# denix56/SI-Mamba

Measured on AMD Instinct MI355X. Metric: point-clouds/sec (fwd+bwd), higher is better.
Workload: dtype f32; 1 GPU; PointMamba classifier train step (FPS+kNN grouping, encoder, spectral SAST ordering, 12 Mamba blocks d=384 at L=1024, head, AdamW), 1024 pts -> 128 patches; global_batch=64, per_gpu_batch=64, npoints=1024, patches=128, mamba_seq_len=1024, parallelism=dp1, communicator_ranks=1, library_gemm=tuned solution table (si_mamba_amd/tuned/gemm_gfx950.csv)

## Files before the change

### include/simamba.h

```cpp
#ifndef SIMAMBA_H_
#define SIMAMBA_H_

#include <stddef.h>

#ifdef __cplusplus
extern "C" {
#endif

#define SIMAMBA_ABI_VERSION 9

#define SIMAMBA_F32  0
#define SIMAMBA_BF16 1

#define SIMAMBA_OK            0
#define SIMAMBA_E_NULLPTR    -1
#define SIMAMBA_E_SHAPE      -2
#define SIMAMBA_E_DTYPE      -3
#define SIMAMBA_E_DSTATE     -4
#define SIMAMBA_E_WIDTH      -5
#define SIMAMBA_E_WORKSPACE  -6
#define SIMAMBA_E_GROUPS     -7
#define SIMAMBA_E_ALIGN      -8
#define SIMAMBA_E_VARIANT    -9

#define SIMAMBA_SCAN_CHUNK 128

#define SIMAMBA_SCAN_CKPT_ROW 128
#define SIMAMBA_SCAN_CKPT_SEQ 16

int         simamba_abi_version(void);
const char* simamba_strerror(int rc);
int         simamba_scan_num_chunks(int seqlen);
int         simamba_scan_fwd_auto_variant(int batch, int dim);
int         simamba_scan_ckpt_step(int batch, int dim, int seqlen, int dstate, int io_dtype);
long long   simamba_scan_ckpt_floats(int batch, int dim, int seqlen, int dstate, int ckpt_step);

#define SIMAMBA_SCAN_AUTO    0
#define SIMAMBA_SCAN_ROWSCAN 1
#define SIMAMBA_SCAN_LPC2    2
#define SIMAMBA_SCAN_LPC4    4
#define SIMAMBA_SCAN_MIX     6
int simamba_selective_scan_fwd(const void* u, const void* delta, const float* A,
                               const void* B, const void* C, const float* D, const void* z,
                               const float* delta_bias, void* out, float* x_ckpt,
                               float* last_state, int batch, int dim, int seqlen, int dstate,
                               int io_dtype, int delta_softplus, long long z_bstride,
                               long long bc_bstride, long long bc_nstride, long long bc_tstride,
                               int ckpt_step, int variant, void* stream);

int simamba_selective_scan_bwd(const void* u, const void* delta, const float* A,
                               const void* B, const void* C, const float* D, const void* z,
                               const float* delta_bias, const void* dout, const float* x_ckpt,
                               void* du, void* ddelta, float* dA, float* dB, float* dC,
                               float* dD, void* dz, float* ddelta_bias,
                               int batch, int dim, int seqlen, int dstate,
                               int io_dtype, int delta_softplus, long long z_bstride,
                               long long dz_bstride, long long bc_bstride, long long bc_nstride,
                               long long bc_tstride, int ckpt_step, void* stream);

int simamba_selective_scan_dt_fwd(const void* u, const void* xdbl, const void* wdt, const float* A, const float* D,
                                  const void* z, const float* delta_bias, void* out, float* x_ckpt, float* last_state,
                                  int batch, int dim, int seqlen, int dstate, int dt_rank, int io_dtype,
                                  long long z_bstride, long long xdbl_bstride, long long xdbl_tstride, int ckpt_step,
                                  int variant, void* stream);
int simamba_selective_scan_dt_bwd(const void* u, const void* xdbl, const void* wdt, const float* A, const float* D,
                                  const void* z, const float* delta_bias, const void* dout, const float* x_ckpt,
                                  void* du, void* ddelta, float* dA, float* dB, float* dC, float* dD, void* dz,
                                  float* ddelta_bias, int batch, int dim, int seqlen, int dstate, int dt_rank,
                                  int io_dtype, long long z_bstride, long long dz_bstride, long long xdbl_bstride,
                                  long long xdbl_tstride, void* stream);

int simamba_xdt_proj_fwd(const void* x, const void* wx, const void* wdt, void* xdbl, void* delta,
                         int batch, int D, int seqlen, int S, int R, int io_dtype, long long x_bstride,
                         void* stream);
int simamba_conv_xdt_proj_fwd(const void* x, const float* cw, const float* cb, const void* wx, const void* wdt,
                              void* xconv, void* xdbl, void* delta, int batch, int D, int seqlen, int S, int R,
                              int io_dtype, long long x_bstride, void* stream);

int simamba_seq_gather_fwd(const void* in, const int* idx, void* out, int batch, int channels, int G, int L,
                           long long out_bstride, int io_dtype, void* stream);
int simamba_seq_gather_bwd(const void* dout, const int* inv, void* din, int batch, int channels, int G, int L,
                           int R, long long dout_bstride, int io_dtype, void* stream);

int simamba_causal_conv1d_fwd(const void* x, const float* w, const float* bias, void* out,
                              int batch, int dim, int seqlen, int width, int silu,
                              int io_dtype, long long x_bstride, void* stream);
int simamba_causal_conv1d_bwd(const void* x, const float* w, const float* bias,
                              const void* dout, void* dx, float* dw, float* dbias,
                              int batch, int dim, int seqlen, int width, int silu,
                              int io_dtype, long long x_bstride, long long dx_bstride, void* stream);

int simamba_add_layer_norm_grid(int batch, int rows_per_batch);
int simamba_add_layer_norm_fwd(const void* hidden, const float* residual, const float* rowscale,
                               const float* weight, const float* bias, float* residual_out,
                               void* normed, float* mean, float* rstd, int batch, int rows_per_batch,
                               int dim, float eps, int hidden_dtype, int out_dtype, void* stream);
int simamba_add_layer_norm_bwd(const void* dnormed, const float* dresidual_out,
                               const float* residual_out, const float* mean, const float* rstd,
                               const float* weight, const float* rowscale, float* dresidual,
                               void* dhidden, float* dwb_partial, int batch, int rows_per_batch,
                               int dim, int hidden_dtype, int out_dtype, void* stream);

int simamba_out_proj_add_ln_fwd(const void* y, const void* w, const float* residual, const float* rowscale,
                                const float* gamma, const float* beta, float* residual_out, void* normed, float* mean,
                                float* rstd, int batch, int K, int L, int C, float eps, int out_dtype, void* stream);

int simamba_in_proj_fwd(const void* x, const void* w, void* xz, int batch, int L, int C, int M, int io_dtype,
                        void* stream);

int simamba_bn_relu_grid(long long rows);
int simamba_bn_relu_fwd(const void* x, const float* gterm, int group, const float* weight, const float* bias,
                        float* running_mean, float* running_var, float momentum, float eps, int training,
                        void* y, float* mean, float* invstd, float* partial, long long rows, int C,
                        long long ld, int io_dtype, void* stream);
int simamba_bn_relu_bwd(const void* dy, const void* x, const float* gterm, int group, const float* weight,
                        const float* bias, const float* mean, const float* invstd, void* dx, float* dgterm,
                        int dgroup, float* dweight, float* dbias, float* partial, long long rows, int C,
                        long long ld, int io_dtype, int training, void* stream);
int simamba_group_max_fwd(const void* x, void* out, unsigned char* idx, long long groups, int n, int C,
                          int io_dtype, void* stream);
int simamba_group_max_bwd(const void* dout, const unsigned char* idx, void* dx, long long groups, int n, int C,
                          int io_dtype, void* stream);

int simamba_three_nn(const float* xyz1, const float* xyz2, int* idx, float* weight, int batch, int N, int S,
                     void* stream);
int simamba_three_interpolate_fwd(const void* feats, const int* idx, const float* weight, void* out, int batch,
                                  int N, int S, int C, int io_dtype, void* stream);
int simamba_three_interpolate_bwd(const void* dout, const int* idx, const float* weight, float* dfeats, int batch,
                                  int N, int S, int C, int io_dtype, void* stream);

int simamba_chamfer_fwd(const float* pred, const float* gt, float* dist, unsigned char* idx1, unsigned char* idx2,
                        long long pairs, int n, int m, void* stream);
int simamba_chamfer_bwd(const float* pred, const float* gt, const float* ddist, const unsigned char* idx1,
                        const unsigned char* idx2, float* dpred, long long pairs, int n, int m, void* stream);

int simamba_knn_group(const float* points, const float* centers, long long* idx, int batch, int N, int G, int K,
                      void* stream);

#define SIMAMBA_SPEC_SYMMETRIC   0x01u
#define SIMAMBA_SPEC_SELF_LOOP   0x02u
#define SIMAMBA_SPEC_BINARY      0x04u
#define SIMAMBA_SPEC_MATRIX_SYM  0x08u
#define SIMAMBA_SPEC_SMALLEST    0x10u
#define SIMAMBA_SPEC_SIGMA_MEAN  0x20u

int simamba_knn_graph(const float* points, float* adj, void* workspace, size_t ws_bytes,
                      int B, int G, int F, int knn, float alpha, unsigned flags, void* stream);

int simamba_laplacian_topk(const float* adj, float* evals, float* evecs, long long* order,
                           float* all_evals, float* all_evecs, int B, int G, int k,
                           unsigned flags, void* stream);

size_t simamba_spectral_workspace_bytes(int B, int G);

int simamba_spectral_topk(const float* centers, float* evals, float* evecs, long long* order,
                          void* workspace, size_t ws_bytes, int B, int G, int knn, float alpha,
                          int k, unsigned flags, void* stream);

int simamba_farthest_point_sample(const float* points, long long* idx, float* centers, int B, int N,
                                  int K, void* stream);

int simamba_argsort_rows(const float* vals, long long* idx, int rows, int n, void* stream);

#ifdef __cplusplus
}
#endif
#endif
```

### si_mamba_amd/_lib.py

```python
from __future__ import annotations

import ctypes
import os
from ctypes import c_char_p, c_float, c_int, c_longlong, c_size_t, c_uint, c_void_p

_HERE = os.path.dirname(os.path.abspath(__file__))
LIB_PATH = os.path.join(_HERE, "libsimamba_hip.so")

F32, BF16 = 0, 1

SPEC_SYMMETRIC = 0x01
SPEC_SELF_LOOP = 0x02
SPEC_BINARY = 0x04
SPEC_MATRIX_SYM = 0x08
SPEC_SMALLEST = 0x10
SPEC_SIGMA_MEAN = 0x20

SCAN_AUTO, SCAN_ROWSCAN, SCAN_LPC2, SCAN_LPC4, SCAN_MIX = 0, 1, 2, 4, 6
CKPT_ROW, CKPT_SEQ = 128, 16

_P = c_void_p
_LL = c_longlong
ABI_VERSION = 9
SIGNATURES = {
    "simamba_abi_version": (c_int, []),
    "simamba_strerror": (c_char_p, [c_int]),
    "simamba_scan_num_chunks": (c_int, [c_int]),
    "simamba_scan_fwd_auto_variant": (c_int, [c_int, c_int]),
    "simamba_scan_ckpt_step": (c_int, [c_int, c_int, c_int, c_int, c_int]),
    "simamba_scan_ckpt_floats": (_LL, [c_int, c_int, c_int, c_int, c_int]),
    "simamba_selective_scan_fwd": (c_int, [_P, _P, _P, _P, _P, _P, _P, _P, _P, _P, _P,
                                           c_int, c_int, c_int, c_int, c_int, c_int,
                                           _LL, _LL, _LL, _LL, c_int, c_int, _P]),
    "simamba_selective_scan_bwd": (c_int, [_P, _P, _P, _P, _P, _P, _P, _P, _P, _P,
                                           _P, _P, _P, _P, _P, _P, _P, _P,
                                           c_int, c_int, c_int, c_int, c_int, c_int,
                                           _LL, _LL, _LL, _LL, _LL, c_int, _P]),
    "simamba_selective_scan_dt_fwd": (c_int, [_P, _P, _P, _P, _P, _P, _P, _P, _P, _P,
                                              c_int, c_int, c_int, c_int, c_int, c_int,
                                              _LL, _LL, _LL, c_int, c_int, _P]),
    "simamba_selective_scan_dt_bwd": (c_int, [_P, _P, _P, _P, _P, _P, _P, _P, _P,
                                              _P, _P, _P, _P, _P, _P, _P, _P,
                                              c_int, c_int, c_int, c_int, c_int, c_int,
                                              _LL, _LL, _LL, _LL, _P]),
    "simamba_xdt_proj_fwd": (c_int, [_P, _P, _P, _P, _P, c_int, c_int, c_int, c_int, c_int, c_int, _LL, _P]),
    "simamba_conv_xdt_proj_fwd": (c_int, [_P, _P, _P, _P, _P, _P, _P, _P, c_int, c_int, c_int, c_int, c_int, c_int, _LL,
                                          _P]),
    "simamba_seq_gather_fwd": (c_int, [_P, _P, _P, c_int, c_int, c_int, c_int, _LL, c_int, _P]),
    "simamba_seq_gather_bwd": (c_int, [_P, _P, _P, c_int, c_int, c_int, c_int, c_int, _LL, c_int, _P]),
    "simamba_causal_conv1d_fwd": (c_int, [_P, _P, _P, _P, c_int, c_int, c_int, c_int, c_int, c_int, _LL, _P]),
    "simamba_causal_conv1d_bwd": (c_int, [_P, _P, _P, _P, _P, _P, _P,
                                          c_int, c_int, c_int, c_int, c_int, c_int, _LL, _LL, _P]),
    "simamba_add_layer_norm_grid": (c_int, [c_int, c_int]),
    "simamba_add_layer_norm_fwd": (c_int, [_P, _P, _P, _P, _P, _P, _P, _P, _P, c_int, c_int, c_int, c_float,
                                           c_int, c_int, _P]),
    "simamba_add_layer_norm_bwd": (c_int, [_P, _P, _P, _P, _P, _P, _P, _P, _P, _P, c_int, c_int, c_int,
                                           c_int, c_int, _P]),
    "simamba_out_proj_add_ln_fwd": (c_int, [_P, _P, _P, _P, _P, _P, _P, _P, _P, _P, c_int, c_int, c_int, c_int, c_float,
                                            c_int, _P]),
    "simamba_in_proj_fwd": (c_int, [_P, _P, _P, c_int, c_int, c_int, c_int, c_int, _P]),
    "simamba_bn_relu_grid": (c_int, [_LL]),
    "simamba_bn_relu_fwd": (c_int, [_P, _P, c_int, _P, _P, _P, _P, c_float, c_float, c_int, _P, _P, _P, _P, _LL, c_int,
                                    _LL, c_int, _P]),
    "simamba_bn_relu_bwd": (c_int, [_P, _P, _P, c_int, _P, _P, _P, _P, _P, _P, c_int, _P, _P, _P, _LL, c_int, _LL,
                                    c_int, c_int, _P]),
    "simamba_group_max_fwd": (c_int, [_P, _P, _P, _LL, c_int, c_int, c_int, _P]),
    "simamba_group_max_bwd": (c_int, [_P, _P, _P, _LL, c_int, c_int, c_int, _P]),
    "simamba_three_nn": (c_int, [_P, _P, _P, _P, c_int, c_int, c_int, _P]),
    "simamba_three_interpolate_fwd": (c_int, [_P, _P, _P, _P, c_int, c_int, c_int, c_int, c_int, _P]),
    "simamba_three_interpolate_bwd": (c_int, [_P, _P, _P, _P, c_int, c_int, c_int, c_int, c_int, _P]),
    "simamba_chamfer_fwd": (c_int, [_P, _P, _P, _P, _P, _LL, c_int, c_int, _P]),
    "simamba_chamfer_bwd": (c_int, [_P, _P, _P, _P, _P, _P, _LL, c_int, c_int, _P]),
    "simamba_knn_group": (c_int, [_P, _P, _P, c_int, c_int, c_int, c_int, _P]),
    "simamba_knn_graph": (c_int, [_P, _P, _P, c_size_t, c_int, c_int, c_int, c_int, c_float, c_uint, _P]),
    "simamba_laplacian_topk": (c_int, [_P, _P, _P, _P, _P, _P, c_int, c_int, c_int, c_uint, _P]),
    "simamba_spectral_workspace_bytes": (c_size_t, [c_int, c_int]),
    "simamba_spectral_topk": (c_int, [_P, _P, _P, _P, _P, c_size_t, c_int, c_int, c_int, c_float,
                                      c_int, c_uint, _P]),
    "simamba_argsort_rows": (c_int, [_P, _P, c_int, c_int, _P]),
    "simamba_farthest_point_sample": (c_int, [_P, _P, _P, c_int, c_int, c_int, _P]),
}

_lib = None


def load():
    global _lib
    if _lib is not None:
        return _lib
    if not os.path.exists(LIB_PATH):
        raise RuntimeError(
            f"{LIB_PATH} not found: build it with `python -c 'import __graft_entry__ as g; g.build()'` "
            "or `make -C si_mamba_amd/csrc`.  si_mamba_amd has no CPU / eager fallback.")
    lib = ctypes.CDLL(LIB_PATH)
    for name, (res, args) in SIGNATURES.items():
        fn = getattr(lib, name)
        fn.restype = res
        fn.argtypes = args
    got = lib.simamba_abi_version()
    if got != ABI_VERSION:
        raise RuntimeError(f"libsimamba_hip.so ABI version {got}, binding expects {ABI_VERSION}")
    _lib = lib
    return lib


def check(rc: int, what: str):
    if rc != 0:
        msg = load().simamba_strerror(rc).decode()
        raise RuntimeError(f"{what} failed (rc={rc}): {msg}")


def ptr(t):
    return None if t is None else t.data_ptr()


def dtype_code(dtype):
    import torch
    if dtype == torch.float32:
        return F32
    if dtype == torch.bfloat16:
        return BF16
    raise TypeError(f"si_mamba_amd kernels take float32 or bfloat16 activations, got {dtype}")


def stream_ptr(device):
    import torch
    return torch.cuda.current_stream(device).cuda_stream


def require_gpu(t, what):
    if not t.is_cuda:
        raise RuntimeError(
            f"{what}: tensor is on {t.device}; si_mamba_amd runs on a ROCm device only "
            "(no CPU fallback -- the CPU restatement lives in oracle/ and is test-only)")


_timing = {"on": False, "events": {}, "only": None}


def enable_kernel_timing(on=True, only=None):
    _timing["on"] = bool(on)
    _timing["events"] = {}
    _timing["only"] = None if only is None else frozenset(only)


class timed:
    __slots__ = ("name", "dev", "ev")

    def __init__(self, name, device):
        self.name, self.dev, self.ev = name, device, None

    def __enter__(self):
        if _timing["on"] and (_timing["only"] is None or self.name in _timing["only"]):
            import torch
            a, b = torch.cuda.Event(enable_timing=True), torch.cuda.Event(enable_timing=True)
            a.record(torch.cuda.current_stream(self.dev))
            self.ev = (a, b)
        return self

    def __exit__(self, *exc):
        if self.ev is not None:
            import torch
            self.ev[1].record(torch.cuda.current_stream(self.dev))
            _timing["events"].setdefault(self.name, []).append(self.ev)
        return False


def kernel_times():
    out = {}
    for name, evs in _timing["events"].items():
        ms = [a.elapsed_time(b) for a, b in evs]
        out[name] = (len(ms), sum(ms) / max(len(ms), 1))
    return out


_scan_variant = [SCAN_AUTO]


class scan_variant:

    def __init__(self, variant):
        self.v, self.prev = int(variant), None

    def __enter__(self):
        self.prev, _scan_variant[0] = _scan_variant[0], self.v
        return self

    def __exit__(self, *exc):
        _scan_variant[0] = self.prev
        return False


def current_scan_variant():
    return _scan_variant[0]


_scan_ckpt = [0]


class scan_ckpt:

    def __init__(self, step):
        self.v, self.prev = int(step), None

    def __enter__(self):
        self.prev, _scan_ckpt[0] = _scan_ckpt[0], self.v
        return self

    def __exit__(self, *exc):
        _scan_ckpt[0] = self.prev
        return False


_fuse_dt = [None]
counters = {}


def count(name):
    counters[name] = counters.get(name, 0) + 1



class scan_fuse_dt:

    def __init__(self, on):
        self.v, self.prev = (None if on is None else bool(on)), None

    def __enter__(self):
        self.prev, _fuse_dt[0] = _fuse_dt[0], self.v
        return self

    def __exit__(self, *exc):
        _fuse_dt[0] = self.prev
        return False


def fuse_dt_enabled(dtype):
    import torch
    return (dtype == torch.bfloat16) if _fuse_dt[0] is None else _fuse_dt[0]


_fuse_out_norm = [True]
_hand_in_proj = [None]


class fuse_out_norm:

    def __init__(self, on):
        self.v, self.prev = bool(on), None

    def __enter__(self):
        self.prev, _fuse_out_norm[0] = _fuse_out_norm[0], self.v
        return self

    def __exit__(self, *exc):
        _fuse_out_norm[0] = self.prev
        return False


def fuse_out_norm_enabled():
    return _fuse_out_norm[0]


class hand_in_proj:

    def __init__(self, on):
        self.v, self.prev = (None if on is None else bool(on)), None

    def __enter__(self):
        self.prev, _hand_in_proj[0] = _hand_in_proj[0], self.v
        return self

    def __exit__(self, *exc):
        _hand_in_proj[0] = self.prev
        return False


def in_proj_hand_enabled(workgroups, dtype=None):
    import torch
    if _hand_in_proj[0] is not None:
        return _hand_in_proj[0]
    return dtype != torch.float32 and workgroups >= IN_PROJ_MIN_WORKGROUPS


IN_PROJ_MIN_WORKGROUPS = 192


def scan_plan(batch, dim, seqlen, dstate, dtype, aligned, device, need_grad):
    import torch
    lib = load()
    code = dtype_code(dtype)
    step = _scan_ckpt[0] or lib.simamba_scan_ckpt_step(batch, dim, seqlen, dstate, code)
    if step == CKPT_SEQ and not (aligned and dstate == 16 and dim % 64 == 0 and
                                 seqlen % (4 if code == F32 else 8) == 0):
        step = CKPT_ROW
    if _scan_variant[0] == SCAN_ROWSCAN:
        step = CKPT_ROW
    if not need_grad:
        return step, None
    n = lib.simamba_scan_ckpt_floats(batch, dim, seqlen, dstate, step)
    return step, (torch.empty(n, device=device, dtype=torch.float32) if n else None)


def scan_bwd_accumulators(batch, dim, seqlen, dstate, has_D, has_bias, device):
    import torch
    sizes = [dim * dstate, batch * dstate * seqlen, batch * dstate * seqlen, dim if has_D else 0,
             dim if has_bias else 0]
    flat = torch.empty(sum(sizes), device=device, dtype=torch.float32)
    parts, o = [], 0
    for n in sizes:
        parts.append(flat[o:o + n])
        o += n
    dA = parts[0].view(dim, dstate)
    dB = parts[1].view(batch, dstate, seqlen)
    dC = parts[2].view(batch, dstate, seqlen)
    return dA, dB, dC, (parts[3] if has_D else None), (parts[4] if has_bias else None)
```

### si_mamba_amd/mamba_inner.py

```python
from __future__ import annotations

import torch

from . import _lib


def _w(t, dtype):
    return t if t.dtype == dtype else t.to(dtype)


def _wx(W, X):
    return torch.bmm(W.unsqueeze(0).expand(X.shape[0], -1, -1), X)


def _xw(X, W):
    return torch.bmm(X, W.unsqueeze(0).expand(X.shape[0], -1, -1))


def _sum_bmm(X, Y):
    return torch.bmm(X, Y).sum(0, dtype=torch.float32)


class InProjFn(torch.autograd.Function):

    @staticmethod
    def forward(ctx, hidden, weight, bias):
        io = hidden.dtype
        if torch.is_autocast_enabled("cuda"):
            io = torch.get_autocast_dtype("cuda")
            hidden = hidden.to(io)
        wc = _w(weight, io)
        xz = tokens_times_weight(hidden, wc) if bias is None else _wx(wc, hidden.transpose(1, 2))
        if bias is not None:
            xz = xz + _w(bias, io)[None, :, None]
        ctx.save_for_backward(hidden, weight)
        ctx.wc = wc
        ctx.has_bias = bias is not None
        return xz

    @staticmethod
    def backward(ctx, dxz):
        hidden, weight = ctx.saved_tensors
        io = hidden.dtype
        dxz = dxz.to(io)
        dh = _xw(dxz.transpose(1, 2), ctx.wc) if ctx.needs_input_grad[0] else None
        dw = _sum_bmm(dxz, hidden).to(weight.dtype) if ctx.needs_input_grad[1] else None
        db = dxz.sum((0, 2)).to(weight.dtype) if ctx.has_bias else None
        return dh, dw, db


def tokens_times_weight(x, w):
    if (x.dtype in (torch.bfloat16, torch.float32) and w.dtype == x.dtype and x.is_cuda and x.dim() == 3
            and x.is_contiguous() and in_proj_hand_ok(x, w)):
        lib = _lib.load()
        Bsz, L, C = x.shape
        wcc = w.contiguous()
        out = torch.empty(Bsz, w.shape[0], L, device=x.device, dtype=x.dtype)
        with torch.cuda.device(x.device), _lib.timed("in_proj_fwd", x.device):
            rc = lib.simamba_in_proj_fwd(x.data_ptr(), wcc.data_ptr(), out.data_ptr(), Bsz, L, C, w.shape[0],
                                         _lib.dtype_code(x.dtype), _lib.stream_ptr(x.device))
        _lib.check(rc, "simamba_in_proj_fwd")
        _lib.count("in_proj_hand")
        return out
    return _wx(w, x.transpose(1, 2))


def in_proj_hand_ok(hidden, wc):
    Bsz, L, C = hidden.shape
    tile = 128 if hidden.dtype == torch.float32 else 256
    return (C % 64 == 0 and C <= 384 and wc.shape[0] % 32 == 0 and L % 8 == 0 and hidden.data_ptr() % 16 == 0
            and _lib.in_proj_hand_enabled(Bsz * ((L + tile - 1) // tile), hidden.dtype))


def in_proj_fn(hidden, weight, bias=None):
    return InProjFn.apply(hidden, weight, bias)


def xdt_proj_fused_ok(x, wx, wdt, conv=False):
    S, D = wx.shape
    R = wdt.shape[1]
    pack = 4 if x.dtype == torch.float32 else 8
    return (x.is_cuda and x.dtype in (torch.float32, torch.bfloat16) and wx.dtype == x.dtype and wdt.dtype == x.dtype
            and x.dim() == 3 and x.stride(2) == 1 and x.stride(1) == x.shape[2] and x.stride(0) % pack == 0
            and x.shape[1] == D and D % 64 == 0 and x.shape[2] % pack == 0 and S % 4 == 0 and S <= 64
            and D * x.shape[2] * 4 < 2 ** 32 - 65536 and (not conv or D <= 1024)
            and R % 4 == 0 and 4 <= R <= 24 and S >= R and wdt.shape[0] == D and x.data_ptr() % 16 == 0)


def xdt_proj_fwd(x, wx, wdt, conv=None, want_delta=True):
    lib = _lib.load()
    Bsz, D, L = x.shape
    S, R = wx.shape[0], wdt.shape[1]
    wxc, wdc = wx.contiguous(), wdt.contiguous()
    x_dbl = torch.empty(Bsz, L, S, device=x.device, dtype=x.dtype)
    delta = torch.empty(Bsz, D, L, device=x.device, dtype=x.dtype) if want_delta else None
    with torch.cuda.device(x.device), _lib.timed("xdt_proj_fwd", x.device):
        if conv is None:
            rc = lib.simamba_xdt_proj_fwd(x.data_ptr(), wxc.data_ptr(), wdc.data_ptr(), x_dbl.data_ptr(),
                                          _lib.ptr(delta), Bsz, D, L, S, R, _lib.dtype_code(x.dtype), x.stride(0),
                                          _lib.stream_ptr(x.device))
        else:
            cw, cb, out = conv
            rc = lib.simamba_conv_xdt_proj_fwd(x.data_ptr(), cw.data_ptr(), _lib.ptr(cb), wxc.data_ptr(), wdc.data_ptr(),
                                               out.data_ptr(), x_dbl.data_ptr(), _lib.ptr(delta), Bsz, D, L, S, R,
                                               _lib.dtype_code(x.dtype), x.stride(0), _lib.stream_ptr(x.device))
    _lib.check(rc, "simamba_xdt_proj_fwd")
    return x_dbl, delta


class MambaInnerFn(torch.autograd.Function):
    @staticmethod
    def forward(ctx, xz, conv_w, conv_b, x_proj_w, dt_proj_w, out_proj_w, out_proj_b, A, D, delta_bias,
                dt_rank, d_state, grad_mode=True):
        _lib.require_gpu(xz, "mamba_inner_fn")
        lib = _lib.load()
        if xz.stride(2) != 1 or xz.stride(1) != xz.shape[2]:
            xz = xz.contiguous()
        io = xz.dtype
        code = _lib.dtype_code(io)
        Bsz, twoD, L = xz.shape
        Dm = twoD // 2
        R, N = dt_rank, d_state
        S = R + 2 * N
        dev = xz.device
        stream = _lib.stream_ptr(dev)
        xbs = xz.stride(0)
        x_in, z = xz[:, :Dm], xz[:, Dm:]

        cw = conv_w.float().contiguous()
        cb = None if conv_b is None else conv_b.float().contiguous()
        Af = A.float().contiguous()
        Df = None if D is None else D.float().contiguous()
        bf = None if delta_bias is None else delta_bias.float().contiguous()
        W = cw.shape[1]

        no_out = out_proj_w is None
        xw_c, dtw_c = _w(x_proj_w, io), _w(dt_proj_w, io)
        ow_c = None if no_out else _w(out_proj_w, io)
        ctx.wcast = (xw_c, dtw_c, ow_c)
        x_conv = torch.empty(Bsz, Dm, L, device=dev, dtype=io)
        need_grad = grad_mode and any(ctx.needs_input_grad)
        pack = 4 if io == torch.float32 else 8
        aligned = xz.data_ptr() % 16 == 0 and (xbs * xz.element_size()) % 16 == 0
        ckpt_step, x_ckpt = _lib.scan_plan(Bsz, Dm, L, N, io, aligned, dev, need_grad)
        fuse_dt = (_lib.fuse_dt_enabled(io) and ckpt_step == _lib.CKPT_SEQ and N == 16 and R % pack == 0 and R <= 24
                   and _lib.current_scan_variant() != _lib.SCAN_ROWSCAN)
        if W == 4 and xdt_proj_fused_ok(x_in, xw_c, dtw_c, conv=True):
            x_dbl, delta = xdt_proj_fwd(x_in, xw_c, dtw_c, conv=(cw, cb, x_conv), want_delta=not fuse_dt)
        else:
            fuse_dt = False
            with torch.cuda.device(dev), _lib.timed("conv1d_fwd", dev):
                rc = lib.simamba_causal_conv1d_fwd(x_in.data_ptr(), cw.data_ptr(), _lib.ptr(cb), x_conv.data_ptr(),
                                                   Bsz, Dm, L, W, 1, code, xbs, stream)
            _lib.check(rc, "simamba_causal_conv1d_fwd")
            if xdt_proj_fused_ok(x_conv, xw_c, dtw_c):
                x_dbl, delta = xdt_proj_fwd(x_conv, xw_c, dtw_c)
            else:
                x_dbl = _xw(x_conv.transpose(1, 2), xw_c.t())
                delta = _wx(dtw_c, x_dbl[:, :, :R].transpose(1, 2))
        Bv, Cv = x_dbl[:, :, R:R + N], x_dbl[:, :, R + N:]
        if x_dbl.data_ptr() % 16:
            raise RuntimeError("mamba_inner_fn: unaligned x_proj output")

        y = torch.empty(Bsz, Dm, L, device=dev, dtype=io)
        dtw_k = dtw_c.contiguous() if fuse_dt else None
        with torch.cuda.device(dev), _lib.timed("scan_fwd", dev):
            if fuse_dt:
                _lib.count("scan_dt_fwd")
                rc = lib.simamba_selective_scan_dt_fwd(
                    x_conv.data_ptr(), x_dbl.data_ptr(), dtw_k.data_ptr(), Af.data_ptr(), _lib.ptr(Df),
                    z.data_ptr(), _lib.ptr(bf), y.data_ptr(), _lib.ptr(x_ckpt), None,
                    Bsz, Dm, L, N, R, code, xbs, x_dbl.stride(0), x_dbl.stride(1),
                    ckpt_step, _lib.current_scan_variant(), stream)
            else:
                rc = lib.simamba_selective_scan_fwd(
                    x_conv.data_ptr(), delta.data_ptr(), Af.data_ptr(), Bv.data_ptr(), Cv.data_ptr(), _lib.ptr(Df),
                    z.data_ptr(), _lib.ptr(bf), y.data_ptr(), _lib.ptr(x_ckpt), None,
                    Bsz, Dm, L, N, code, 1, xbs, x_dbl.stride(0), 1, x_dbl.stride(1),
                    ckpt_step, _lib.current_scan_variant(), stream)
        _lib.check(rc, "simamba_selective_scan_fwd")

        if no_out:
            out = y
        else:
            out = _xw(y.transpose(1, 2), ow_c.t())
            if out_proj_b is not None:
                out = out + _w(out_proj_b, io)
        ctx.no_out = no_out
        ctx.dims = (R, N, W)
        ctx.ckpt_step = ckpt_step
        ctx.dtw_k = dtw_k
        ctx.has_out_bias = out_proj_b is not None and not no_out
        ctx.param_dtypes = (conv_w.dtype, None if conv_b is None else conv_b.dtype, x_proj_w.dtype,
                            dt_proj_w.dtype, None if no_out else out_proj_w.dtype, A.dtype,
                            None if D is None else D.dtype, None if delta_bias is None else delta_bias.dtype)
        ctx.save_for_backward(xz, x_conv, x_dbl, delta, None if no_out else y, cw, cb, x_proj_w, dt_proj_w, out_proj_w,
                              Af, Df, bf, x_ckpt)
        return out

    @staticmethod
    def backward(ctx, dout):
        (xz, x_conv, x_dbl, delta, y, cw, cb, x_proj_w, dt_proj_w, out_proj_w, Af, Df, bf, x_ckpt) = ctx.saved_tensors
        lib = _lib.load()
        R, N, W = ctx.dims
        io = xz.dtype
        code = _lib.dtype_code(io)
        Bsz, twoD, L = xz.shape
        Dm = twoD // 2
        S = R + 2 * N
        dev = xz.device
        stream = _lib.stream_ptr(dev)
        xbs = xz.stride(0)
        dout = dout.to(io)
        f32 = dict(device=dev, dtype=torch.float32)
        xw_c, dtw_c, ow_c = ctx.wcast
        if ctx.no_out:
            dy = dout.contiguous()
            d_out_w = d_out_b = None
        else:
            if dout.stride(2) != 1:
                dout = dout.contiguous()
            d_out_w = _sum_bmm(dout.transpose(1, 2), y.transpose(1, 2))
            d_out_b = dout.sum((0, 1)) if ctx.has_out_bias else None
            dy = tokens_times_weight(dout, ow_c.t())

        dxz = torch.empty_like(xz)
        du = torch.empty(Bsz, Dm, L, device=dev, dtype=io)
        ddelta = torch.empty(Bsz, Dm, L, device=dev, dtype=io)
        dA, dB, dC, dD, dbias = _lib.scan_bwd_accumulators(Bsz, Dm, L, N, Df is not None, bf is not None, dev)
        Bv, Cv = x_dbl[:, :, R:R + N], x_dbl[:, :, R + N:]
        z, dz = xz[:, Dm:], dxz[:, Dm:]
        with torch.cuda.device(dev), _lib.timed("scan_bwd", dev):
            if ctx.dtw_k is not None:
                rc = lib.simamba_selective_scan_dt_bwd(
                    x_conv.data_ptr(), x_dbl.data_ptr(), ctx.dtw_k.data_ptr(), Af.data_ptr(), _lib.ptr(Df),
                    z.data_ptr(), _lib.ptr(bf), dy.data_ptr(), _lib.ptr(x_ckpt),
                    du.data_ptr(), ddelta.data_ptr(), dA.data_ptr(), dB.data_ptr(), dC.data_ptr(), _lib.ptr(dD),
                    dz.data_ptr(), _lib.ptr(dbias), Bsz, Dm, L, N, R, code,
                    xbs, dxz.stride(0), x_dbl.stride(0), x_dbl.stride(1), stream)
            else:
                rc = lib.simamba_selective_scan_bwd(
                    x_conv.data_ptr(), delta.data_ptr(), Af.data_ptr(), Bv.data_ptr(), Cv.data_ptr(), _lib.ptr(Df),
                    z.data_ptr(), _lib.ptr(bf), dy.data_ptr(), _lib.ptr(x_ckpt),
                    du.data_ptr(), ddelta.data_ptr(), dA.data_ptr(), dB.data_ptr(), dC.data_ptr(), _lib.ptr(dD),
                    dz.data_ptr(), _lib.ptr(dbias), Bsz, Dm, L, N, code, 1,
                    xbs, dxz.stride(0), x_dbl.stride(0), 1, x_dbl.stride(1), ctx.ckpt_step, stream)
        _lib.check(rc, "simamba_selective_scan_bwd")

        dx_dbl = torch.empty(Bsz, L, S, device=dev, dtype=io)
        dx_dbl[:, :, :R].copy_(_xw(ddelta.transpose(1, 2), dtw_c))
        dBC = torch.as_strided(dB, (2, Bsz, N, L), (Bsz * N * L, N * L, L, 1))
        dx_dbl[:, :, R:].view(Bsz, L, 2, N).copy_(dBC.permute(1, 3, 0, 2))
        d_dt_w = _sum_bmm(ddelta, x_dbl[:, :, :R])
        d_x_w = _sum_bmm(dx_dbl.transpose(1, 2), x_conv.transpose(1, 2))
        wxT = xw_c.t().unsqueeze(0).expand(Bsz, -1, -1)
        torch.baddbmm(du, wxT, dx_dbl.transpose(1, 2), out=du)

        dconv = torch.empty(Dm * W + (Dm if cb is not None else 0), **f32)
        dcw = dconv[:Dm * W].view(Dm, W)
        dcb = dconv[Dm * W:] if cb is not None else None
        with torch.cuda.device(dev), _lib.timed("conv1d_bwd", dev):
            rc = lib.simamba_causal_conv1d_bwd(xz.data_ptr(), cw.data_ptr(), _lib.ptr(cb), du.data_ptr(),
                                               dxz.data_ptr(), dcw.data_ptr(), _lib.ptr(dcb),
                                               Bsz, Dm, L, W, 1, code, xbs, dxz.stride(0), stream)
        _lib.check(rc, "simamba_causal_conv1d_bwd")

        t_cw, t_cb, t_xw, t_dtw, t_ow, t_A, t_D, t_b = ctx.param_dtypes
        return (dxz, dcw.to(t_cw), None if dcb is None else dcb.to(t_cb), d_x_w.to(t_xw), d_dt_w.to(t_dtw),
                None if d_out_w is None else d_out_w.to(t_ow),
                None if d_out_b is None else d_out_b.to(out_proj_w.dtype), dA.to(t_A),
                None if dD is None else dD.to(t_D), None if dbias is None else dbias.to(t_b), None, None, None)


def mamba_inner_fn(xz, conv1d_weight, conv1d_bias, x_proj_weight, delta_proj_weight, out_proj_weight,
                   out_proj_bias, A, D=None, delta_bias=None, dt_rank=None, d_state=None):
    if conv1d_weight.dim() == 3:
        conv1d_weight = conv1d_weight.squeeze(1)
    if dt_rank is None:
        dt_rank = delta_proj_weight.shape[1]
    if d_state is None:
        d_state = (x_proj_weight.shape[0] - dt_rank) // 2
    return MambaInnerFn.apply(xz, conv1d_weight, conv1d_bias, x_proj_weight, delta_proj_weight, out_proj_weight,
                              out_proj_bias, A, D, delta_bias, dt_rank, d_state, torch.is_grad_enabled())
```

Before: 1119 point-clouds/s.

## Fuse x_proj backward GEMMs with causal conv1d backward into one HIP kernel

Adds a fused f32 HIP kernel that computes the x_proj input-gradient GEMM on MFMA, adds it to du, and applies the SiLU and causal conv1d backward to produce dx, dconv weight and bias. In the same pass it recomputes the conv output to accumulate per-batch x_proj weight-gradient partials, which a small follow-up kernel reduces. This replaces two batched GEMMs, the x_conv read and a separate conv1d backward launch, cutting launches and round trips of du through memory. The cost is recomputing the conv forward inside the kernel, a per-batch partial buffer, and atomics for the conv gradients.

```diff
diff --git a/include/simamba.h b/include/simamba.h
--- a/include/simamba.h
+++ b/include/simamba.h
@@ -76,6 +76,11 @@
 int simamba_conv_xdt_proj_fwd(const void* x, const float* cw, const float* cb, const void* wx, const void* wdt,
                               void* xconv, void* xdbl, void* delta, int batch, int D, int seqlen, int S, int R,
                               int io_dtype, long long x_bstride, void* stream);
+
+int simamba_xproj_conv_bwd(const void* x, const float* cw, const float* cb, const void* wx, const void* du,
+                           const void* g, void* dx, float* dxw_part, float* dxw, float* dcw, float* dcb,
+                           int batch, int D, int seqlen, int S, int io_dtype, long long x_bstride,
+                           long long dx_bstride, void* stream);
 
 int simamba_seq_gather_fwd(const void* in, const int* idx, void* out, int batch, int channels, int G, int L,
                            long long out_bstride, int io_dtype, void* stream);
diff --git a/si_mamba_amd/_lib.py b/si_mamba_amd/_lib.py
--- a/si_mamba_amd/_lib.py
+++ b/si_mamba_amd/_lib.py
@@ -46,6 +46,8 @@
     "simamba_xdt_proj_fwd": (c_int, [_P, _P, _P, _P, _P, c_int, c_int, c_int, c_int, c_int, c_int, _LL, _P]),
     "simamba_conv_xdt_proj_fwd": (c_int, [_P, _P, _P, _P, _P, _P, _P, _P, c_int, c_int, c_int, c_int, c_int, c_int, _LL,
                                           _P]),
+    "simamba_xproj_conv_bwd": (c_int, [_P, _P, _P, _P, _P, _P, _P, _P, _P, _P, _P, c_int, c_int, c_int, c_int, c_int,
+                                       _LL, _LL, _P]),
     "simamba_seq_gather_fwd": (c_int, [_P, _P, _P, c_int, c_int, c_int, c_int, _LL, c_int, _P]),
     "simamba_seq_gather_bwd": (c_int, [_P, _P, _P, c_int, c_int, c_int, c_int, c_int, _LL, c_int, _P]),
     "simamba_causal_conv1d_fwd": (c_int, [_P, _P, _P, _P, c_int, c_int, c_int, c_int, c_int, c_int, _LL, _P]),
@@ -240,6 +242,27 @@
     return (dtype == torch.bfloat16) if _fuse_dt[0] is None else _fuse_dt[0]
 
 
+_fuse_xproj_conv_bwd = [True]
+
+
+class fuse_xproj_conv_bwd:
+
+    def __init__(self, on):
+        self.v, self.prev = bool(on), None
+
+    def __enter__(self):
+        self.prev, _fuse_xproj_conv_bwd[0] = _fuse_xproj_conv_bwd[0], self.v
+        return self
+
+    def __exit__(self, *exc):
+        _fuse_xproj_conv_bwd[0] = self.prev
+        return False
+
+
+def fuse_xproj_conv_bwd_enabled():
+    return _fuse_xproj_conv_bwd[0]
+
+
 _fuse_out_norm = [True]
 _hand_in_proj = [None]
 
diff --git a/si_mamba_amd/csrc/xdt_proj_bwd.hip b/si_mamba_amd/csrc/xdt_proj_bwd.hip
--- /dev/null
+++ b/si_mamba_amd/csrc/xdt_proj_bwd.hip
@@ -0,0 +1,324 @@
+#include "common.h"
+
+namespace simamba {
+
+typedef float f32x16 __attribute__((ext_vector_type(16)));
+
+constexpr int kXbThreads = 256;
+constexpr int kXbTok = 64;
+constexpr int kXbCh = 64;
+constexpr int kXbP = kXbTok + 4;
+constexpr int kXbKH = 28;
+constexpr unsigned kXbOob = 0xfffff000u;
+
+using xb_rsrc_t = __amdgpu_buffer_rsrc_t;
+
+__device__ __forceinline__ xb_rsrc_t xb_rsrc(const void* base, unsigned bytes) {
+  return __builtin_amdgcn_make_buffer_rsrc(const_cast<void*>(base), 0, static_cast<int>(bytes), 0x00020000);
+}
+using xb_vec4_t = decltype(__builtin_amdgcn_raw_buffer_load_b128(xb_rsrc(nullptr, 0u), 0u, 0u, 0));
+__device__ __forceinline__ float4 xb_load4(xb_rsrc_t r, unsigned voff, unsigned soff) {
+  return __builtin_bit_cast(float4, __builtin_amdgcn_raw_buffer_load_b128(r, voff, soff, 0));
+}
+__device__ __forceinline__ void xb_store4(float4 f, xb_rsrc_t r, unsigned voff, unsigned soff) {
+  __builtin_amdgcn_raw_buffer_store_b128(__builtin_bit_cast(xb_vec4_t, f), r, voff, soff, 0);
+}
+
+struct XbArgs {
+  const float* x;
+  const float* cw;
+  const float* cb;
+  const float* wx;
+  const float* du;
+  const float* g;
+  float* dx;
+  float* part;
+  float* dcw;
+  float* dcb;
+  int batch, D, L, S;
+  long long x_bs, dx_bs;
+};
+
+__global__ __launch_bounds__(kXbThreads, 2) void xproj_conv_bwd_f32_kernel(XbArgs p) {
+  __shared__ __attribute__((aligned(16))) float sGT[64 * kXbP];
+  __shared__ __attribute__((aligned(16))) float sDxc[kXbCh * kXbP];
+  __shared__ __attribute__((aligned(16))) float sWx[2 * kXbKH * kXbCh];
+  const int tid = threadIdx.x;
+  const int lane = tid & 63;
+  const int wave = __builtin_amdgcn_readfirstlane(tid >> 6);
+  const int li = lane & 31, hh = lane >> 5;
+  const int D = p.D, L = p.L, S = p.S;
+  const int d0 = static_cast<int>(blockIdx.x) * kXbCh;
+  const int b = static_cast<int>(blockIdx.y);
+  const int ntiles = (L + kXbTok - 1) / kXbTok;
+  const int S4 = S >> 2;
+
+  for (int i = tid; i < 64 * kXbP; i += kXbThreads) sGT[i] = 0.f;
+  __syncthreads();
+
+  const int pd = tid >> 2, seg = tid & 3;
+  const int dg = d0 + pd;
+  float w4[4];
+  {
+    const float4 t4 = *reinterpret_cast<const float4*>(p.cw + 4 * static_cast<size_t>(dg));
+    w4[0] = t4.x; w4[1] = t4.y; w4[2] = t4.z; w4[3] = t4.w;
+  }
+  const float bias = p.cb ? p.cb[dg] : 0.f;
+
+  const unsigned sample_bytes = static_cast<unsigned>(D) * static_cast<unsigned>(L) * 4u;
+  const xb_rsrc_t rs_x = xb_rsrc(p.x + static_cast<size_t>(b) * p.x_bs, sample_bytes);
+  const xb_rsrc_t rs_du = xb_rsrc(p.du + static_cast<size_t>(b) * D * L, sample_bytes);
+  const xb_rsrc_t rs_dx = xb_rsrc(p.dx + static_cast<size_t>(b) * p.dx_bs, sample_bytes);
+  const xb_rsrc_t rs_g = xb_rsrc(p.g + static_cast<size_t>(b) * L * S, static_cast<unsigned>(L) * S * 4u);
+  const unsigned row_off = (static_cast<unsigned>(dg) * L + 16u * seg) * 4u;
+
+  int gt[4], gs4[4];
+#pragma unroll
+  for (int k = 0; k < 4; ++k) {
+    const int i = tid + kXbThreads * k;
+    gt[k] = i / (S4 > 0 ? S4 : 1);
+    gs4[k] = i - gt[k] * S4;
+    if (gt[k] >= kXbTok) gt[k] = -1;
+  }
+
+  for (int i = tid; i < 2 * kXbKH * kXbCh; i += kXbThreads) {
+    const int s = i / kXbCh, d = i - s * kXbCh;
+    sWx[i] = s < S ? p.wx[static_cast<size_t>(s) * D + d0 + d] : 0.f;
+  }
+  const int p1d = 32 * (wave & 1), p1t = 32 * (wave >> 1);
+  const int p2s = 32 * (wave & 1), p2d = 32 * (wave >> 1);
+  f32x16 acc2;
+#pragma unroll
+  for (int r = 0; r < 16; ++r) acc2[r] = 0.f;
+
+  struct Loads { float4 x[4], du[4], g[4]; };
+  auto issue = [&](Loads& ld, int tile) {
+    const int t0 = __builtin_amdgcn_readfirstlane(tile * kXbTok);
+    const bool live = tile < ntiles;
+#pragma unroll
+    for (int k = 0; k < 4; ++k) {
+      const bool ok = live && t0 + 16 * seg + 4 * k < L;
+      const unsigned v = ok ? row_off + 16u * k + 4u * t0 : kXbOob;
+      ld.x[k] = xb_load4(rs_x, v, 0u);
+      ld.du[k] = xb_load4(rs_du, v, 0u);
+      const bool gok = live && gt[k] >= 0 && gs4[k] < S4 && t0 + gt[k] < L;
+      ld.g[k] = xb_load4(rs_g, gok ? 16u * (tid + kXbThreads * k) + 4u * t0 * S : kXbOob, 0u);
+    }
+  };
+
+  float gw[4] = {0.f, 0.f, 0.f, 0.f}, gb = 0.f;
+  float xprev[3] = {0.f, 0.f, 0.f};
+  float dprev[16];
+#pragma unroll
+  for (int i = 0; i < 16; ++i) dprev[i] = 0.f;
+
+  auto emit_dx = [&](int tile, const float (&nxt)[3]) {
+    float dp[19];
+#pragma unroll
+    for (int i = 0; i < 16; ++i) dp[i] = dprev[i];
+#pragma unroll
+    for (int i = 0; i < 3; ++i) dp[16 + i] = nxt[i];
+    const int t0 = __builtin_amdgcn_readfirstlane(tile * kXbTok);
+#pragma unroll
+    for (int k = 0; k < 4; ++k) {
+      float o[4];
+#pragma unroll
+      for (int i = 0; i < 4; ++i) {
+        float acc = 0.f;
+#pragma unroll
+        for (int j = 0; j < 4; ++j) acc = fmaf(w4[j], dp[4 * k + i + 3 - j], acc);
+        o[i] = acc;
+      }
+      const bool ok = t0 + 16 * seg + 4 * k < L;
+      xb_store4(make_float4(o[0], o[1], o[2], o[3]), rs_dx, ok ? row_off + 16u * k + 4u * t0 : kXbOob, 0u);
+    }
+  };
+
+  Loads cur;
+  issue(cur, 0);
+  for (int tile = 0; tile < ntiles; ++tile) {
+#pragma unroll
+    for (int k = 0; k < 4; ++k) {
+      if (gt[k] >= 0 && gs4[k] < S4) {
+        const float4 v = cur.g[k];
+        const int c = 4 * gs4[k] * kXbP + gt[k];
+        sGT[c] = v.x; sGT[c + kXbP] = v.y; sGT[c + 2 * kXbP] = v.z; sGT[c + 3 * kXbP] = v.w;
+      }
+    }
+    __syncthreads();
+
+    {
+      f32x16 acc;
+#pragma unroll
+      for (int r = 0; r < 16; ++r) acc[r] = 0.f;
+#pragma unroll 4
+      for (int m = 0; m < kXbKH; ++m)
+        acc = __builtin_amdgcn_mfma_f32_32x32x2f32(sWx[(hh * kXbKH + m) * kXbCh + p1d + li], sGT[(hh * kXbKH + m) * kXbP + p1t + li], acc, 0, 0, 0);
+#pragma unroll
+      for (int r = 0; r < 16; ++r) sDxc[(p1d + (r & 3) + 8 * (r >> 2) + 4 * hh) * kXbP + p1t + li] = acc[r];
+    }
+    __syncthreads();
+
+    float xv[16], duv[16];
+#pragma unroll
+    for (int k = 0; k < 4; ++k) {
+      xv[4 * k] = cur.x[k].x; xv[4 * k + 1] = cur.x[k].y; xv[4 * k + 2] = cur.x[k].z; xv[4 * k + 3] = cur.x[k].w;
+      duv[4 * k] = cur.du[k].x; duv[4 * k + 1] = cur.du[k].y; duv[4 * k + 2] = cur.du[k].z; duv[4 * k + 3] = cur.du[k].w;
+    }
+    float xw[19];
+    {
+      float h[3];
+#pragma unroll
+      for (int i = 0; i < 3; ++i) {
+        const float nb = __shfl(xv[13 + i], lane - 1);
+        h[i] = seg == 0 ? xprev[i] : nb;
+      }
+#pragma unroll
+      for (int i = 0; i < 3; ++i) xw[i] = (tile == 0 && seg == 0) ? 0.f : h[i];
+#pragma unroll
+      for (int i = 0; i < 16; ++i) xw[3 + i] = xv[i];
+    }
+    {
+      float nx[3];
+#pragma unroll
+      for (int i = 0; i < 3; ++i) nx[i] = __shfl(xv[13 + i], lane + 3);
+#pragma unroll
+      for (int i = 0; i < 3; ++i) xprev[i] = nx[i];
+    }
+    float* dxrow = &sDxc[pd * kXbP + 16 * seg];
+    float dpre[16];
+#pragma unroll
+    for (int k = 0; k < 4; ++k) {
+      const float4 v = *reinterpret_cast<const float4*>(dxrow + 4 * k);
+      const float y[4] = {v.x, v.y, v.z, v.w};
+      float xc[4];
+#pragma unroll
+      for (int i = 0; i < 4; ++i) {
+        const int n = 4 * k + i;
+        float pre = bias;
+#pragma unroll
+        for (int j = 0; j < 4; ++j) pre = fmaf(w4[j], xw[n + j], pre);
+        const float sg = sigmoid_f(pre);
+        xc[i] = pre * sg;
+        const float gdx = duv[n] + y[i];
+        dpre[n] = gdx * sg * (1.f + pre * (1.f - sg));
+        gb += dpre[n];
+#pragma unroll
+        for (int j = 0; j < 4; ++j) gw[j] = fmaf(dpre[n], xw[n + j], gw[j]);
+      }
+      *reinterpret_cast<float4*>(dxrow + 4 * k) = make_float4(xc[0], xc[1], xc[2], xc[3]);
+    }
+    if (tile > 0) {
+      float nxt[3];
+#pragma unroll
+      for (int i = 0; i < 3; ++i) {
+        const float a = __shfl(dprev[i], lane + 1);
+        const float c = __shfl(dpre[i], lane - 3);
+        nxt[i] = seg == 3 ? c : a;
+      }
+      emit_dx(tile - 1, nxt);
+    }
+#pragma unroll
+    for (int i = 0; i < 16; ++i) dprev[i] = dpre[i];
+    issue(cur, tile + 1);
+    __syncthreads();
+
+    {
+      const float* ga = &sGT[(p2s + li) * kXbP + 32 * hh];
+      const float* xb = &sDxc[(p2d + li) * kXbP + 32 * hh];
+#pragma unroll 2
+      for (int q = 0; q < 8; ++q) {
+        const float4 av = *reinterpret_cast<const float4*>(ga + 4 * q);
+        const float4 bv = *reinterpret_cast<const float4*>(xb + 4 * q);
+        acc2 = __builtin_amdgcn_mfma_f32_32x32x2f32(av.x, bv.x, acc2, 0, 0, 0);
+        acc2 = __builtin_amdgcn_mfma_f32_32x32x2f32(av.y, bv.y, acc2, 0, 0, 0);
+        acc2 = __builtin_amdgcn_mfma_f32_32x32x2f32(av.z, bv.z, acc2, 0, 0, 0);
+        acc2 = __builtin_amdgcn_mfma_f32_32x32x2f32(av.w, bv.w, acc2, 0, 0, 0);
+      }
+    }
+    __syncthreads();
+  }
+
+  if (ntiles > 0) {
+    float nxt[3];
+#pragma unroll
+    for (int i = 0; i < 3; ++i) {
+      const float a = __shfl(dprev[i], lane + 1);
+      nxt[i] = seg == 3 ? 0.f : a;
+    }
+    emit_dx(ntiles - 1, nxt);
+  }
+
+  float* part = p.part + static_cast<size_t>(b) * S * D + d0 + p2d + li;
+#pragma unroll
+  for (int r = 0; r < 16; ++r) {
+    const int s = p2s + (r & 3) + 8 * (r >> 2) + 4 * hh;
+    if (s < S) part[static_cast<size_t>(s) * D] = acc2[r];
+  }
+
+#pragma unroll
+  for (int j = 0; j < 4; ++j) {
+    gw[j] += __shfl_xor(gw[j], 1);
+    gw[j] += __shfl_xor(gw[j], 2);
+  }
+  gb += __shfl_xor(gb, 1);
+  gb += __shfl_xor(gb, 2);
+  if (seg == 0) {
+#pragma unroll
+    for (int j = 0; j < 4; ++j) atomicAdd(&p.dcw[4 * dg + j], gw[j]);
+    if (p.dcb) atomicAdd(&p.dcb[dg], gb);
+  }
+}
+
+__global__ __launch_bounds__(256) void xproj_wgrad_sum_kernel(const float* __restrict__ part, float* __restrict__ out,
+                                                              int batch, int n) {
+  const int i = static_cast<int>(blockIdx.x) * 256 + static_cast<int>(threadIdx.x);
+  if (i >= n) return;
+  float acc = 0.f;
+  for (int b = 0; b < batch; ++b) acc += part[static_cast<size_t>(b) * n + i];
+  out[i] = acc;
+}
+
+}
+
+using namespace simamba;
+
+extern "C" int simamba_xproj_conv_bwd(const void* x, const float* cw, const float* cb, const void* wx, const void* du,
+                                      const void* g, void* dx, float* dxw_part, float* dxw, float* dcw, float* dcb,
+                                      int batch, int D, int L, int S, int io_dtype, long long x_bstride,
+                                      long long dx_bstride, void* stream) {
+  if (batch < 0 || D <= 0 || L < 0 || S <= 0 || batch > 65535) return SIMAMBA_E_SHAPE;
+  if (io_dtype != SIMAMBA_F32) return SIMAMBA_E_DTYPE;
+  if (D % kXbCh || L % 4 || S % 4 || S > 2 * kXbKH) return SIMAMBA_E_SHAPE;
+  if (static_cast<long long>(D) * L * 4 >= (1LL << 32) - 65536 || static_cast<long long>(L) * S * 4 >= (1LL << 31))
+    return SIMAMBA_E_SHAPE;
+  if (!x || !cw || !wx || !du || !g || !dx || !dxw_part || !dxw || !dcw) return SIMAMBA_E_NULLPTR;
+  const uintptr_t al = reinterpret_cast<uintptr_t>(x) | reinterpret_cast<uintptr_t>(cw) |
+                       reinterpret_cast<uintptr_t>(wx) | reinterpret_cast<uintptr_t>(du) |
+                       reinterpret_cast<uintptr_t>(g) | reinterpret_cast<uintptr_t>(dx);
+  if (al & 15u) return SIMAMBA_E_ALIGN;
+  XbArgs a{};
+  a.x = static_cast<const float*>(x); a.cw = cw; a.cb = cb; a.wx = static_cast<const float*>(wx);
+  a.du = static_cast<const float*>(du); a.g = static_cast<const float*>(g); a.dx = static_cast<float*>(dx);
+  a.part = dxw_part; a.dcw = dcw; a.dcb = dcb;
+  a.batch = batch; a.D = D; a.L = L; a.S = S;
+  a.x_bs = x_bstride ? x_bstride : static_cast<long long>(D) * L;
+  a.dx_bs = dx_bstride ? dx_bstride : static_cast<long long>(D) * L;
+  if (a.x_bs % 4 || a.dx_bs % 4) return SIMAMBA_E_ALIGN;
+  hipStream_t s = static_cast<hipStream_t>(stream);
+  const bool joined = dcb == dcw + static_cast<size_t>(D) * 4;
+  hipError_t e = hipMemsetAsync(dcw, 0, sizeof(float) * (static_cast<size_t>(D) * 4 + (joined ? D : 0)), s);
+  if (e != hipSuccess) return static_cast<int>(e);
+  if (dcb && !joined) {
+    e = hipMemsetAsync(dcb, 0, sizeof(float) * D, s);
+    if (e != hipSuccess) return static_cast<int>(e);
+  }
+  const int n = S * D;
+  if (batch == 0 || L == 0) {
+    e = hipMemsetAsync(dxw, 0, sizeof(float) * n, s);
+    return static_cast<int>(e);
+  }
+  hipLaunchKernelGGL(xproj_conv_bwd_f32_kernel, dim3(D / kXbCh, batch), dim3(kXbThreads), 0, s, a);
+  hipLaunchKernelGGL(xproj_wgrad_sum_kernel, dim3((n + 255) / 256), dim3(256), 0, s, dxw_part, dxw, batch, n);
+  return static_cast<int>(hipGetLastError());
+}
diff --git a/si_mamba_amd/mamba_inner.py b/si_mamba_amd/mamba_inner.py
--- a/si_mamba_amd/mamba_inner.py
+++ b/si_mamba_amd/mamba_inner.py
@@ -85,6 +85,17 @@
             and x.shape[1] == D and D % 64 == 0 and x.shape[2] % pack == 0 and S % 4 == 0 and S <= 64
             and D * x.shape[2] * 4 < 2 ** 32 - 65536 and (not conv or D <= 1024)
             and R % 4 == 0 and 4 <= R <= 24 and S >= R and wdt.shape[0] == D and x.data_ptr() % 16 == 0)
+
+
+def xproj_conv_bwd_ok(xz, dxz, wx, W, R, N):
+    Bsz, twoD, L = xz.shape
+    Dm = twoD // 2
+    S = R + 2 * N
+    return (_lib.fuse_xproj_conv_bwd_enabled() and xz.dtype == torch.float32 and wx.dtype == torch.float32
+            and W == 4 and R <= 24 and N == 16 and S % 4 == 0 and Dm % 64 == 0 and L % 4 == 0 and 0 < Bsz <= 65535
+            and Dm * L * 4 < 2 ** 32 - 65536 and xz.stride(2) == 1 and xz.stride(1) == L and xz.stride(0) % 4 == 0
+            and dxz.stride(2) == 1 and dxz.stride(1) == L and dxz.stride(0) % 4 == 0
+            and xz.data_ptr() % 16 == 0 and dxz.data_ptr() % 16 == 0)
 
 
 def xdt_proj_fwd(x, wx, wdt, conv=None, want_delta=True):
@@ -252,18 +263,30 @@
         dBC = torch.as_strided(dB, (2, Bsz, N, L), (Bsz * N * L, N * L, L, 1))
         dx_dbl[:, :, R:].view(Bsz, L, 2, N).copy_(dBC.permute(1, 3, 0, 2))
         d_dt_w = _sum_bmm(ddelta, x_dbl[:, :, :R])
-        d_x_w = _sum_bmm(dx_dbl.transpose(1, 2), x_conv.transpose(1, 2))
-        wxT = xw_c.t().unsqueeze(0).expand(Bsz, -1, -1)
-        torch.baddbmm(du, wxT, dx_dbl.transpose(1, 2), out=du)
-
         dconv = torch.empty(Dm * W + (Dm if cb is not None else 0), **f32)
         dcw = dconv[:Dm * W].view(Dm, W)
         dcb = dconv[Dm * W:] if cb is not None else None
-        with torch.cuda.device(dev), _lib.timed("conv1d_bwd", dev):
-            rc = lib.simamba_causal_conv1d_bwd(xz.data_ptr(), cw.data_ptr(), _lib.ptr(cb), du.data_ptr(),
-                                               dxz.data_ptr(), dcw.data_ptr(), _lib.ptr(dcb),
-                                               Bsz, Dm, L, W, 1, code, xbs, dxz.stride(0), stream)
-        _lib.check(rc, "simamba_causal_conv1d_bwd")
+        if xproj_conv_bwd_ok(xz, dxz, xw_c, W, R, N):
+            xwc = xw_c.contiguous()
+            part = torch.empty(Bsz, S, Dm, **f32)
+            d_x_w = torch.empty(S, Dm, **f32)
+            with torch.cuda.device(dev), _lib.timed("xproj_conv_bwd", dev):
+                rc = lib.simamba_xproj_conv_bwd(xz.data_ptr(), cw.data_ptr(), _lib.ptr(cb), xwc.data_ptr(),
+                                                du.data_ptr(), dx_dbl.data_ptr(), dxz.data_ptr(), part.data_ptr(),
+                                                d_x_w.data_ptr(), dcw.data_ptr(), _lib.ptr(dcb), Bsz, Dm, L, S, code,
+                                                xbs, dxz.stride(0), stream)
+            _lib.check(rc, "simamba_xproj_conv_bwd")
+            _lib.count("xproj_conv_bwd")
+        else:
+            d_x_w = _sum_bmm(dx_dbl.transpose(1, 2), x_conv.transpose(1, 2))
+            wxT = xw_c.t().unsqueeze(0).expand(Bsz, -1, -1)
+            torch.baddbmm(du, wxT, dx_dbl.transpose(1, 2), out=du)
+
+            with torch.cuda.device(dev), _lib.timed("conv1d_bwd", dev):
+                rc = lib.simamba_causal_conv1d_bwd(xz.data_ptr(), cw.data_ptr(), _lib.ptr(cb), du.data_ptr(),
+                                                   dxz.data_ptr(), dcw.data_ptr(), _lib.ptr(dcb),
+                                                   Bsz, Dm, L, W, 1, code, xbs, dxz.stride(0), stream)
+            _lib.check(rc, "simamba_causal_conv1d_bwd")
 
         t_cw, t_cb, t_xw, t_dtw, t_ow, t_A, t_D, t_b = ctx.param_dtypes
         return (dxz, dcw.to(t_cw), None if dcb is None else dcb.to(t_cb), d_x_w.to(t_xw), d_dt_w.to(t_dtw),
```

Measured after the change: 1123 point-clouds/s (median of 6 runs). No clear change (+0.4%).
